# NOAA-GFDL/pace

Hardware: AMD Instinct MI355X
Metric: simulated-days/day + acoustic-step ms, C768 L79 fp64, 1/2/4/8 MI355X (higher is better)
Workload: dtype f64

## Files before the change

### pace_amd/csrc/fv3_common.h

```cpp
#pragma once
#include <type_traits>
#include <algorithm>

#include <cmath>
#include <cstdint>
#include <cstdio>
#include <cstdlib>
#include <cstring>
#include <string>
#include <vector>

#include "../../include/fv3_mi355x.h"
#include "fv3_switch.h"

#ifdef FV3_HOST_EMU
#define FV3_HD
#define FV3_DEV
typedef void *fv3_stream_t;
#else
#include <hip/hip_runtime.h>
#define FV3_HD __host__ __device__
#define FV3_DEV __device__
typedef hipStream_t fv3_stream_t;
#endif

#ifndef FV3_REAL
#define FV3_REAL double
#endif
typedef FV3_REAL Real;

#if defined(FV3_STAMPS) && !defined(FV3_HOST_EMU)
#define FV3_STAMP_RECS 16384
unsigned long long *fv3_stamp_buf();
#if defined(__HIP_DEVICE_COMPILE__)
#define FV3_STAMP_STATE unsigned st_t = (unsigned)__builtin_amdgcn_s_memtime(), st_a[6] = {0u, 0u, 0u, 0u, 0u, 0u}, st_n = 0u
#define FV3_STAMP(i)                                            \
  do {                                                          \
    __builtin_amdgcn_sched_barrier(0);                          \
    const unsigned t_ = (unsigned)__builtin_amdgcn_s_memtime(); \
    st_a[i] += t_ - st_t;                                       \
    st_t = t_;                                                  \
    if ((i) == 0) ++st_n;                                       \
    __builtin_amdgcn_sched_barrier(0);                          \
  } while (0)
#define FV3_STAMP_USE(x) asm volatile("" ::"v"(x))
#define FV3_STAMP_FLUSH(buf, kid, tid)                                          \
  do {                                                                          \
    if ((tid) == 0 && ((buf)[1] == 0ull || (buf)[1] == (kid))) {                \
      const unsigned long long slot_ = atomicAdd((buf), 1ull);                  \
      if (slot_ < FV3_STAMP_RECS) {                                             \
        unsigned long long *r_ = (buf) + 8 + slot_ * 8;                         \
        r_[0] = (kid);                                                          \
        r_[1] = st_n;                                                           \
        for (int q_ = 0; q_ < 6; ++q_) r_[2 + q_] = st_a[q_];                   \
      }                                                                         \
    }                                                                           \
  } while (0)
#else
inline void fv3_stamp_touch(unsigned long long *, unsigned long long, int) {}
#define FV3_STAMP_STATE unsigned st_n = 0u
#define FV3_STAMP(i) ((void)0)
#define FV3_STAMP_USE(x) ((void)0)
// ... 660 lines not shown
#endif
  }
  FV3_HD inline void group_sync() const {
#if !defined(FV3_HOST_EMU) && defined(__HIP_DEVICE_COMPILE__)
    asm volatile("s_waitcnt lgkmcnt(0)\n\ts_barrier" ::: "memory");
#endif
  }
  FV3_HD inline void wave_sync() const {
#if !defined(FV3_HOST_EMU) && defined(__HIP_DEVICE_COMPILE__)
    __builtin_amdgcn_fence(__ATOMIC_RELEASE, "wavefront");
    __builtin_amdgcn_wave_barrier();
    __builtin_amdgcn_fence(__ATOMIC_ACQUIRE, "wavefront");
#endif
  }
};

#ifndef FV3_HOST_EMU
template <class F>
__global__ void __launch_bounds__(256, 2) fv3_kb(GridMap m, F f) {
  extern __shared__ __attribute__((aligned(16))) char fv3_smem[];
  int bx, by, bz;
  if (!fv3_tile(m, bx, by, bz)) return;
  Blk b{(int)threadIdx.x, (int)blockDim.x, bx, by, bz};
  f(b, fv3_smem);
}
#endif

template <class F>
inline void launch_blocks(const fv3_ctx *c, fv3_stream_t s, int gx, int gy, int gz, int nthr, size_t smem_bytes, F f) {
  if (gx <= 0 || gy <= 0 || gz <= 0) return;
#ifdef FV3_HOST_EMU
  (void)c;
  (void)s;
  (void)nthr;
#pragma omp parallel
  {
    std::vector<char> smem(smem_bytes + 16);
#pragma omp for collapse(2) schedule(static)
    for (int z = 0; z < gz; ++z)
      for (int y = 0; y < gy; ++y)
        for (int x = 0; x < gx; ++x) {
          Blk b{0, 1, x, y, z};
          f(b, smem.data());
        }
  }
#else
  (void)c;
  dim3 grid;
  const GridMap m = fv3_grid(gx, gy, gz, &grid);
  hipLaunchKernelGGL(HIP_KERNEL_NAME(fv3_kb<F>), grid, dim3(nthr, 1, 1), smem_bytes, s, m, f);
#endif
}

#define FV3_WAVE 64
#ifdef FV3_HOST_EMU
#define FV3_LPT 64
#define FV3_LANES(blk, lane, l) for (int lane = 0, l = 0; lane < FV3_WAVE; ++lane, ++l)
#else
#define FV3_LPT 1
#define FV3_LANES(blk, lane, l) for (int lane = (blk).tid, l = 0; l < 1; ++l)
template <int WPE, class F>
__global__ void __launch_bounds__(FV3_WAVE) __attribute__((amdgpu_waves_per_eu(WPE, WPE))) fv3_kw(GridMap m, F f) {
  extern __shared__ __attribute__((aligned(16))) char fv3_smem[];
  int bx, by, bz;
  if (!fv3_tile(m, bx, by, bz)) return;
  Blk b{(int)threadIdx.x, FV3_WAVE, bx, by, bz};
  f(b, fv3_smem);
}
#endif

#if !defined(FV3_HOST_EMU) && defined(__HIP_DEVICE_COMPILE__)
FV3_DEV inline int fv3_dpp_shr1_i(int v) { return __builtin_amdgcn_update_dpp(0, v, 0x138, 0xf, 0xf, true); }
FV3_DEV inline int fv3_dpp_shl1_i(int v) { return __builtin_amdgcn_update_dpp(0, v, 0x130, 0xf, 0xf, true); }
FV3_DEV inline double fv3_dpp_shr1(double v) {
  return __hiloint2double(fv3_dpp_shr1_i(__double2hiint(v)), fv3_dpp_shr1_i(__double2loint(v)));
}
FV3_DEV inline double fv3_dpp_shl1(double v) {
  return __hiloint2double(fv3_dpp_shl1_i(__double2hiint(v)), fv3_dpp_shl1_i(__double2loint(v)));
}
FV3_DEV inline float fv3_dpp_shr1(float v) { return __int_as_float(fv3_dpp_shr1_i(__float_as_int(v))); }
FV3_DEV inline float fv3_dpp_shl1(float v) { return __int_as_float(fv3_dpp_shl1_i(__float_as_int(v))); }
template <int K>
FV3_DEV inline Real lane_shr_dev(Real v) {
#pragma unroll
  for (int n = 0; n < K; ++n) v = fv3_dpp_shr1(v);
  return v;
}
template <int K>
FV3_DEV inline Real lane_shl_dev(Real v) {
#pragma unroll
  for (int n = 0; n < K; ++n) v = fv3_dpp_shl1(v);
  return v;
}
#define FV3_LANE_SHR(K, arr, l, lane) lane_shr_dev<K>((arr)[l])
#define FV3_LANE_SHL(K, arr, l, lane) lane_shl_dev<K>((arr)[l])
#else
#define FV3_LANE_SHR(K, arr, l, lane) ((lane) >= (K) ? (arr)[(l) - (K)] : (Real)0)
#define FV3_LANE_SHL(K, arr, l, lane) ((lane) + (K) < FV3_WAVE ? (arr)[(l) + (K)] : (Real)0)
#endif

#ifdef FV3_HOST_EMU
#define FV3_VLPT(CPL) (FV3_WAVE * (CPL))
#define FV3_VLANES(CPL, blk, vl, l) for (int vl = 0; vl < FV3_WAVE * (CPL); ++vl) { const int l = vl; (void)l;
#define FV3_VLANES_END }
#define FV3_VSHR(CPL, K, arr, l, vl) ((vl) >= (K) ? (arr)[(l) - (K)] : (Real)0)
#define FV3_VSHL(CPL, K, arr, l, vl) ((vl) + (K) < FV3_WAVE * (CPL) ? (arr)[(l) + (K)] : (Real)0)
// ... 228 lines not shown
```

### pace_amd/csrc/fv3_dsw.hip

```cpp
#include "fv3_a2b.h"
#include "fv3_ops.h"
#include "fv3_ppm.h"

namespace {

struct FxAdv {
  Geo g;
  const Real *uc, *vc;
  long m2;
  Real dt;
  bool W, E, S, N;

  FV3_HD Real UC(int i, int j) const { return uc[IX(i, j)]; }
  FV3_HD Real VC(int i, int j) const { return vc[IX(i, j)]; }
  FV3_HD Real ut_gen(int i, int j) const {
    return (UC(i, j) - (Real)0.25 * (g.cosa_u + m2)[IX(i, j)] * (VC(i - 1, j) + VC(i, j) + VC(i - 1, j + 1) + VC(i, j + 1))) * (g.rsin_u + m2)[IX(i, j)];
  }
  FV3_HD Real vt_gen(int i, int j) const {
    return (VC(i, j) - (Real)0.25 * (g.cosa_v + m2)[IX(i, j)] * (UC(i, j - 1) + UC(i + 1, j - 1) + UC(i, j) + UC(i + 1, j))) * (g.rsin_v + m2)[IX(i, j)];
  }
  FV3_HD bool edge_col(int i) const { return (W && i == 1) || (E && i == g.npx); }
  FV3_HD bool edge_row(int j) const { return (S && j == 1) || (N && j == g.npy); }
  FV3_HD bool ut_special_row(int j) const { return (S && (j == 0 || j == 1)) || (N && (j == g.npy - 1 || j == g.npy)); }
  FV3_HD Real ut_edge(int i, int j) const {
    const Real u_ = UC(i, j);
    return u_ * dt > (Real)0 ? u_ / (g.sin_sg3 + m2)[IX(i - 1, j)] : u_ / (g.sin_sg1 + m2)[IX(i, j)];
  }
  FV3_HD Real vt_edge(int i, int j) const {
    const Real v_ = VC(i, j);
    return v_ * dt > (Real)0 ? v_ / (g.sin_sg4 + m2)[IX(i, j - 1)] : v_ / (g.sin_sg2 + m2)[IX(i, j)];
  }
  FV3_HD Real ut1(int i, int j) const {
    if (edge_col(i)) return ut_edge(i, j);
    if (ut_special_row(j)) return (Real)0;
    return ut_gen(i, j);
  }
  FV3_HD Real vt1(int i, int j) const {
    if (edge_row(j)) return vt_edge(i, j);
    return vt_gen(i, j);
  }
  FV3_HD bool in_i_rng(int i) const { return i >= (W ? 3 : 1) && i <= (E ? g.npx - 2 : g.nx + 1); }
  FV3_HD bool in_j_rng(int j) const { return j >= (S ? 3 : 1) && j <= (N ? g.npy - 2 : g.ny + 1); }
  FV3_HD bool vt_edge_col(int i) const { return (W && (i == 0 || i == 1)) || (E && (i == g.npx - 1 || i == g.npx)); }
  FV3_HD Real ut2(int i, int j) const {
    if (edge_col(i)) return ut_edge(i, j);
    if (ut_special_row(j)) {
      if (in_i_rng(i))
        return UC(i, j) - (Real)0.25 * (g.cosa_u + m2)[IX(i, j)] * (vt1(i - 1, j) + vt1(i, j) + vt1(i - 1, j + 1) + vt1(i, j + 1));
      return (Real)0;
    }
    return ut_gen(i, j);
  }
  FV3_HD Real vt2(int i, int j) const {
    if (edge_row(j)) return vt_edge(i, j);
    if (vt_edge_col(i) && in_j_rng(j))
// ... 37 lines not shown
    Real s_u = (Real)0;
    for (int n = 0; n < 4; ++n)
      if (!(pbi[n] == it && pbj[n] == j)) s_u = s_u + ut2(pbi[n], pbj[n]);
    const Real cu = (g.cosa_u + m2)[IX(it, j)], cv = (g.cosa_v + m2)[IX(pi, pj)];
    const Real damp = (Real)1 / ((Real)1 - (Real)0.0625 * cu * cv);
    return (UC(it, j) - (Real)0.25 * cu * (s_v + VC(pi, pj) - (Real)0.25 * cv * s_u)) * damp;
  }
  FV3_HD Real vt_corner(int i, int jt, bool west, bool south) const {
    const int npx = g.npx, npy = g.npy;
    const int pj = south ? 1 : npy - 1;
    const int iedge = west ? 1 : npx;
    const int nbi[4] = {i, i + 1, i, i + 1}, nbj[4] = {jt - 1, jt - 1, jt, jt};
    const int pi = (i != iedge) ? i : i + 1;
    Real s_u = (Real)0;
    for (int n = 0; n < 4; ++n)
      if (!(nbi[n] == pi && nbj[n] == pj)) s_u = s_u + ut2(nbi[n], nbj[n]);
    const int pbi[4] = {pi - 1, pi, pi - 1, pi}, pbj[4] = {pj, pj, pj + 1, pj + 1};
    Real s_v = (Real)0;
    for (int n = 0; n < 4; ++n)
      if (!(pbi[n] == i && pbj[n] == jt)) s_v = s_v + vt2(pbi[n], pbj[n]);
    const Real cv = (g.cosa_v + m2)[IX(i, jt)], cu = (g.cosa_u + m2)[IX(pi, pj)];
    const Real damp = (Real)1 / ((Real)1 - (Real)0.0625 * cu * cv);
    return (VC(i, jt) - (Real)0.25 * cv * (s_u + UC(pi, pj) - (Real)0.25 * cu * s_v)) * damp;
  }
  FV3_HD Real ut_final(int i, int j) const {
    bool w_, s_;
    if (ut_corner_target(i, j, w_, s_)) return ut_corner(i, j, w_, s_);
    return ut2(i, j);
  }
  FV3_HD Real vt_final(int i, int j) const {
    bool w_, s_;
    if (vt_corner_target(i, j, w_, s_)) return vt_corner(i, j, w_, s_);
    return vt2(i, j);
  }
};

FV3_HD inline bool fxadv_int_u(const Geo &g, int fl, int i, int j) {
  const bool W = fl & FV3_W, E = fl & FV3_E, S = fl & FV3_S, N = fl & FV3_N;
  return i >= 0 && !((W && i == 1) || (E && i == g.npx)) && !((S && (j == 0 || j == 1)) || (N && (j == g.npy - 1 || j == g.npy)));
}
FV3_HD inline bool fxadv_int_v(const Geo &g, int fl, int i, int j) {
  const bool W = fl & FV3_W, E = fl & FV3_E, S = fl & FV3_S, N = fl & FV3_N;
  return j >= 0 && !((S && j == 1) || (N && j == g.npy)) && !((W && (i == 0 || i == 1)) || (E && (i == g.npx - 1 || i == g.npx)));
}

void fxadv(fv3_ctx *c, fv3_stream_t s, const Real *uc, const Real *vc, Real *crx, Real *cry, Real *xfx, Real *yfx, Real *ut, Real *vt, Real dt, Real *cx,
           Real *cy, bool thin_ut) {
  const Geo g = c->g;
  const bool first = c->seq.acc_first;
  static const bool full_ut = fv3_sw(FV3SW_FXADV_FULL_UT);
  if (full_ut) thin_ut = false;
  const int isd = 1 - g.nh, ied = g.nx + g.nh, jsd = 1 - g.nh, jed = g.ny + g.nh;
  const int npair = (g.nz + FV3_KC - 1) / FV3_KC;
  launch3(c, s, Box{isd, ied, jsd, jed, 0, npair - 1}, [=] FV3_HD(int t, int kp, int i, int j) {
    const int fl = g.flags[t];
    const long m2 = t * g.st2;
    bool int_u = fxadv_int_u(g, fl, i, j), int_v = fxadv_int_v(g, fl, i, j);
    const unsigned p = IX(i, j);
    const bool out_x = int_u && i >= 1 && i <= g.nx + 1, out_y = int_v && j >= 1 && j <= g.ny + 1;
    const bool st_ut = !thin_ut || ((fl & FV3_W) && i <= 4) || ((fl & FV3_E) && i >= g.npx - 3) || ((fl & FV3_S) && j <= 4) || ((fl & FV3_N) && j >= g.npy - 3);
    int_u = int_u && (out_x || st_ut);
    int_v = int_v && (out_y || st_ut);
    if (!int_u && !int_v) return;
    Real cu = 0, ru = 0, rdxa_m = 0, rdxa_0 = 0, dy_ = 0, s3 = 0, s1 = 0;
    Real cv = 0, rv = 0, rdya_m = 0, rdya_0 = 0, dx_ = 0, s4 = 0, s2 = 0;
    if (int_u) {
      cu = (g.cosa_u + m2)[p];
      ru = (g.rsin_u + m2)[p];
    }
    if (out_x) {
      rdxa_m = (g.rdxa + m2)[IX(i - 1, j)];
      rdxa_0 = (g.rdxa + m2)[p];
      dy_ = (g.dy + m2)[p];
      s3 = (g.sin_sg3 + m2)[IX(i - 1, j)];
      s1 = (g.sin_sg1 + m2)[p];
    }
    if (int_v) {
      cv = (g.cosa_v + m2)[p];
      rv = (g.rsin_v + m2)[p];
    }
    if (out_y) {
      rdya_m = (g.rdya + m2)[IX(i, j - 1)];
      rdya_0 = (g.rdya + m2)[p];
      dx_ = (g.dx + m2)[p];
      s4 = (g.sin_sg4 + m2)[IX(i, j - 1)];
      s2 = (g.sin_sg2 + m2)[p];
    }
#ifndef FV3_FXADV_UNROLL
#define FV3_FXADV_UNROLL 1
#endif
#pragma unroll FV3_FXADV_UNROLL
    for (int kk = 0; kk < FV3_KC; ++kk) {
      const int k = FV3_KC * kp + kk;
      if (k > g.nz - 1) break;
      const long b = t * g.st + k * g.sk;
      const Real *ucl = uc + b, *vcl = vc + b;
      if (int_u) {
        const Real utv = (ucl[p] - (Real)0.25 * cu * (vcl[IX(i - 1, j)] + vcl[p] + vcl[IX(i - 1, j + 1)] + vcl[IX(i, j + 1)])) * ru;
        if (st_ut) (ut + b)[p] = utv;
        if (out_x) {
          const Real x = dt * utv;
          Real cr;
          if (x > (Real)0) {
            cr = x * rdxa_m;
            FV3_ST_NT((xfx + b)[p], dy_ * x * s3);
          } else {
            cr = x * rdxa_0;
            FV3_ST_NT((xfx + b)[p], dy_ * x * s1);
          }
          FV3_ST_NT((crx + b)[p], cr);
          if (cx) FV3_ST_NT((cx + b)[p], (first ? (Real)0 : (cx + b)[p]) + cr);
        }
      }
      if (int_v) {
        const Real vtv = (vcl[p] - (Real)0.25 * cv * (ucl[IX(i, j - 1)] + ucl[IX(i + 1, j - 1)] + ucl[p] + ucl[IX(i + 1, j)])) * rv;
        if (st_ut) (vt + b)[p] = vtv;
        if (out_y) {
          const Real y = dt * vtv;
          Real cr;
          if (y > (Real)0) {
            cr = y * rdya_m;
            FV3_ST_NT((yfx + b)[p], dx_ * y * s4);
          } else {
            cr = y * rdya_0;
            FV3_ST_NT((yfx + b)[p], dx_ * y * s2);
          }
          FV3_ST_NT((cry + b)[p], cr);
          if (cy) FV3_ST_NT((cy + b)[p], (first ? (Real)0 : (cy + b)[p]) + cr);
        }
      }
    }
  });
  const int nfr = std::max(ied - isd + 1, jed - jsd + 1);
  launch3(c, s, Box{0, nfr - 1, 1, 8, 0, g.nz - 1}, [=] FV3_HD(int t, int k, int a, int side) {
    const int fl = g.flags[t];
    int i, j;
    if (side <= 4) {
      i = isd + a;
      if (i > ied) return;
      j = side <= 2 ? side - 1 : g.npy - 4 + side;
      if (!(fl & (side <= 2 ? FV3_S : FV3_N))) return;
    } else {
      j = jsd + a;
      if (j > jed) return;
      i = side <= 6 ? side - 5 : g.npx - 8 + side;
      if (!(fl & (side <= 6 ? FV3_W : FV3_E))) return;
      if (((fl & FV3_S) && (j == 0 || j == 1)) || ((fl & FV3_N) && (j == g.npy - 1 || j == g.npy))) return;
    }
    const bool int_u = fxadv_int_u(g, fl, i, j), int_v = fxadv_int_v(g, fl, i, j);
    const long b = t * g.st + k * g.sk, m2 = t * g.st2;
    FxAdv f{g, uc + b, vc + b, m2, dt, (fl & FV3_W) != 0, (fl & FV3_E) != 0, (fl & FV3_S) != 0, (fl & FV3_N) != 0};
    const unsigned p = IX(i, j);
    if (i >= 0 && !int_u) {
      const Real utv = f.ut_final(i, j);
      (ut + b)[p] = utv;
      if (i >= 1 && i <= g.nx + 1) {
        const Real x = dt * utv;
        Real cr;
        if (x > (Real)0) {
          cr = x * (g.rdxa + m2)[IX(i - 1, j)];
          (xfx + b)[p] = (g.dy + m2)[p] * x * (g.sin_sg3 + m2)[IX(i - 1, j)];
        } else {
          cr = x * (g.rdxa + m2)[p];
          (xfx + b)[p] = (g.dy + m2)[p] * x * (g.sin_sg1 + m2)[p];
        }
        (crx + b)[p] = cr;
        if (cx) (cx + b)[p] = (first ? (Real)0 : (cx + b)[p]) + cr;
      }
    }
    if (j >= 0 && !int_v) {
      const Real vtv = f.vt_final(i, j);
      (vt + b)[p] = vtv;
      if (j >= 1 && j <= g.ny + 1) {
        const Real y = dt * vtv;
        Real cr;
        if (y > (Real)0) {
          cr = y * (g.rdya + m2)[IX(i, j - 1)];
          (yfx + b)[p] = (g.dx + m2)[p] * y * (g.sin_sg4 + m2)[IX(i, j - 1)];
        } else {
          cr = y * (g.rdya + m2)[p];
          (yfx + b)[p] = (g.dx + m2)[p] * y * (g.sin_sg2 + m2)[p];
        }
        (cry + b)[p] = cr;
        if (cy) (cy + b)[p] = (first ? (Real)0 : (cy + b)[p]) + cr;
      }
// ... 1097 lines not shown
```

### pace_amd/csrc/fv3_nh.hip

```cpp
#include "fv3_ops.h"
#include "fv3_math.h"
#include "fv3_agpr.h"

#define K_(arr, k) ((arr) + tb + (long)(k)*g.sk)[pix]

namespace {

struct Sim1 {
  Geo g;
  Real rgas, rgrav, p_fac, ptop;
  template <class Setup, class Finish>
  FV3_HD void run(long tb, unsigned pix, Real dt, const Real *delp, const Real *cappa, const Real *pt, const Real *w1, Real ws, Real *PM, Real *DZ, Real *W2, Real *PP,
                  Real *GAM, Real *PE, Real *wout, Setup setup, Finish finish) const {
    const int nz = g.nz;
    const Real t1g = (Real)2.0 * dt * dt, rdt = (Real)1.0 / dt, r3 = (Real)(1.0 / 3.0);
    auto DM = [&](int k) { return K_(delp, k) * rgrav; };
    auto GM = [&](int k) { return (Real)1.0 / ((Real)1.0 - K_(cappa, k)); };
    {
      Real pm_k, dz_k;
      setup(0, pm_k, dz_k);
      Real dm_m = (Real)0, dm_k = DM(0);
      Real pe_k = fv3_exp(GM(0) * fv3_log(-dm_k / dz_k * rgas * K_(pt, 0))) - pm_k;
      Real bet = (Real)0;
      K_(PP, 0) = (Real)0;
// ... 352 lines not shown
        q.v[2] = KW_(cappa, k);
        q.v[3] = KW_(PM, k);
        return q;
      };
      KWALK(4, U, false, ld, {
        const Real dm = r.v[0] * rgrav;
        const Real pe_k = K >= 1 ? A[(K - 1) * FV3_WAVE] : (Real)0;
        if (K == nz - 1) {
          p1 = (pe_k + (Real)2.0 * pe1) * r3;
        } else {
          const Real g_rat = fv3_div(dm, dm_below);
          const Real bb = (Real)2.0 * ((Real)1.0 + g_rat);
          p1 = (pe_k + bb * pe1 + g_rat * pe2) * r3 - g_rat * p1;
        }
        const Real pmk = r.v[3];
        const Real dzn = -dm * rgas * r.v[1] * fv3_exp((r.v[2] - (Real)1.0) * fv3_log(fv3_max(p_fac * pmk, p1 + pmk)));
        cl.finish(K, dzn);
        pe2 = pe1;
        pe1 = pe_k;
        dm_below = dm;
      })
    }
#undef GAM_PUT
#undef GAM_PUT_U
#undef GAM_FLUSH4
  }
};

#ifndef FV3_RIEM_GL
#define FV3_RIEM_GL 0
#endif
inline bool riem_wave_ok(const Geo &g, bool heavy = false) {
  static const int e = fv3_sw(FV3SW_RIEM_MODE);
  if (e == 1) return false;
  const size_t line = (size_t)g.nz * FV3_WAVE * sizeof(Real) * (FV3_RIEM_GL ? 2 : 1);
  if (heavy && e != 2 && line > 40 * 1024) return false;
  if ((g.nz + 2) * g.sk * (long)sizeof(Real) >= (1L << 32)) return false;
  return line <= (FV3_RIEM_GL ? 160 : 64) * 1024 && g.nz >= 3;
}
inline bool riem_gam_lds(const Geo &) { return FV3_RIEM_GL != 0; }
inline bool riem_reg_arrays(const Geo &g) {
  static const bool off = !fv3_sw(FV3SW_RIEM_REGS);
  return !off && !FV3_RIEM_GL && g.nz < (int)FV3_KREG_LEVELS;
}

#ifndef PG_KC
#define PG_KC 16
#endif

struct DzcW {
  Real top_ratio, bot_ratio;
};

}

extern "C" int fv3_update_dz_c(fv3_ctx *c, const fv3_field *zs_, const fv3_field *ut_, const fv3_field *vt_, const fv3_field *gz_, const fv3_field *ws_,
                               double dtd, void *stream) {
  return fv3_update_dz_c_from(c, zs_, ut_, vt_, gz_, gz_, ws_, dtd, stream);
}

int fv3_update_dz_c_from(fv3_ctx *c, const fv3_field *zs_, const fv3_field *ut_, const fv3_field *vt_, const fv3_field *gzin_, const fv3_field *gz_,
                         const fv3_field *ws_, double dtd, void *stream) {
  if (!c) return FV3_ERR_ARG;
  FV3_FIELD2D(zs, zs_) FV3_FIELD(ut, ut_) FV3_FIELD(vt, vt_) FV3_FIELD(gz, gz_) FV3_FIELD(gzin, gzin_) FV3_FIELD2D(ws, ws_)
  const Geo g = c->g;
  fv3_stream_t s = (fv3_stream_t)stream;
  const Real dt = (Real)dtd;
  const int nz = g.nz;
  const Real dz_min = (Real)c->cst.dz_min;
  const std::vector<double> &dp = c->dp_ref_h;
  const Real top_ratio = (Real)(dp[0] / (dp[0] + dp[1]));
  const Real bot_ratio = (Real)(dp[nz - 1] / (dp[nz - 2] + dp[nz - 1]));
  Real *gzn = c->scratch[SC_A];
  if (gzin != gz && nz >= 3) {
    launch2(c, s, Box{0, g.nx + 1, 0, g.ny + 1, 0, 0}, [=] FV3_HD(int t, int i, int j) {
      const int fl = g.flags[t];
      const long tb = t * g.st, m2 = t * g.st2;
      const unsigned pix = IX(i, j), qx1 = IX(i + 1, j), qy1 = IX(i, j + 1);
      const unsigned gw = f4_index<1>(g, fl, i - 1, j), gc1 = f4_index<1>(g, fl, i, j), ge = f4_index<1>(g, fl, i + 1, j);
      const unsigned gs = f4_index<2>(g, fl, i, j - 1), gc2 = f4_index<2>(g, fl, i, j), gn = f4_index<2>(g, fl, i, j + 1);
      const Real ar = (g.area + m2)[pix];
      Real ax0, ax1, ay0, ay1, cx0 = (Real)0, cx1 = (Real)0, cy0 = (Real)0, cy1 = (Real)0, px0 = (Real)0, px1 = (Real)0, py0 = (Real)0, py1 = (Real)0;
      {
        const Real *u1 = ut + tb + (long)(nz - 1) * g.sk, *v1 = vt + tb + (long)(nz - 1) * g.sk;
        ax0 = u1[pix];
        ax1 = u1[qx1];
        ay0 = v1[pix];
        ay1 = v1[qy1];
      }
      Real below = (Real)0;
#pragma unroll 1
      for (int k = nz; k >= 0; --k) {
        Real nx0 = (Real)0, nx1 = (Real)0, ny0 = (Real)0, ny1 = (Real)0;
        if (k >= 2) {
          const Real *u2 = ut + tb + (long)(k - 2) * g.sk, *v2 = vt + tb + (long)(k - 2) * g.sk;
          nx0 = u2[pix];
          nx1 = u2[qx1];
          ny0 = v2[pix];
          ny1 = v2[qy1];
        }
        Real x0, x1, y0, y1;
        if (k == nz) {
          x0 = ax0 + (ax0 - nx0) * bot_ratio;
          x1 = ax1 + (ax1 - nx1) * bot_ratio;
          y0 = ay0 + (ay0 - ny0) * bot_ratio;
          y1 = ay1 + (ay1 - ny1) * bot_ratio;
        } else if (k == 0) {
          x0 = cx0 + (cx0 - px0) * top_ratio;
          x1 = cx1 + (cx1 - px1) * top_ratio;
          y0 = cy0 + (cy0 - py0) * top_ratio;
          y1 = cy1 + (cy1 - py1) * top_ratio;
        } else {
          const Real d1 = g.dp_ref[k], d0 = g.dp_ref[k - 1];
          const Real int_ratio = (Real)1.0 / (d0 + d1);
          x0 = (d1 * ax0 + d0 * cx0) * int_ratio;
          x1 = (d1 * ax1 + d0 * cx1) * int_ratio;
          y0 = (d1 * ay0 + d0 * cy0) * int_ratio;
          y1 = (d1 * ay1 + d0 * cy1) * int_ratio;
        }
        const Real *gg = gzin + tb + (long)k * g.sk;
        const Real fx0 = x0 * (x0 > (Real)0 ? gg[gw] : gg[gc1]);
        const Real fx1 = x1 * (x1 > (Real)0 ? gg[gc1] : gg[ge]);
        const Real fy0 = y0 * (y0 > (Real)0 ? gg[gs] : gg[gc2]);
        const Real fy1 = y1 * (y1 > (Real)0 ? gg[gc2] : gg[gn]);
        const Real zn = (gg[pix] * ar + fx0 - fx1 + fy0 - fy1) / (ar + x0 - x1 + y0 - y1);
        Real v = zn;
        if (k == nz) {
          ws[t * g.st2 + pix] = (zs[t * g.st2 + pix] - zn) / dt;
// ... 1047 lines not shown
```

### pace_amd/csrc/fv3_switch.h

```cpp
#pragma once
#include <atomic>
#include <cstdlib>
#include <cstring>

#define FV3_SW_ONCE true
#define FV3_SW_LIVE false

enum fv3_sw_kind { FV3_SW_present, FV3_SW_off_if_0, FV3_SW_on_if_1, FV3_SW_tri, FV3_SW_word, FV3_SW_integer, FV3_SW_names };

#define FV3_SWITCH_TABLE(X) \
  X(SEG, "FV3_SEG", LIVE, integer, "", 0, "rows a marching wave owns; unset or <= 0 (default): automatic, 96 where that still fills the chip eight times over, else 64") \
  X(GRID_SPLIT, "FV3_GRID_SPLIT", ONCE, off_if_0, "", 0, "0: whole planes per XCD also for launches of few planes; default: such launches map sub-planes to the XCDs") \
  X(FRAME_LAUNCH, "FV3_FRAME_LAUNCH", ONCE, word, "split", 0, "split: one launch per boundary window; default: the four windows of a frame in one launch") \
  X(Q4_KB, "FV3_Q4_KB", ONCE, integer, "", 16, "levels of one tile an XCD walks back to back in the transport marches (level-major launches; default 16); 0: plane-major launches") \
  X(KE_KB, "FV3_KE_KB", ONCE, integer, "", 16, "the same for the corner-KE, divergence-damping and fused wind-stage marches (default 16); 0: plane-major launches") \
  X(GATHER_BATCH, "FV3_GATHER_BATCH", ONCE, off_if_0, "", 0, "0: one launch per halo gather; default: up to twelve gathers per launch") \
  X(AUX_STREAM, "FV3_AUX_STREAM", LIVE, off_if_0, "", 0, "0: everything in program order on the caller's stream; default: small launches on an auxiliary stream beside the marches (read when a context is created)") \
  X(ALT, "FV3_ALT", LIVE, names, "", 0, "named alternatives of the uncertain restatements (DESIGN section 2; the oracle reads the same variable), e.g. dz_damp_scaled,heat_dt_full; default: none") \
  X(DEBUG_FD, "FV3_DEBUG_FD", LIVE, present, "", 0, "set: the operators report on stderr which forms and level ranges they chose; default: silent") \
  X(DEBUG_DEL2, "FV3_DEBUG_DEL2", LIVE, present, "", 0, "set: the fused del2_cubed + heating reports its calls on stderr; default: silent") \
  X(TP2D_MODE, "FV3_TP2D_MODE", ONCE, word, "staged", 0, "staged: fv_tp_2d as one launch per stage (reference path, no auxiliary stream); default: the marching kernels") \
  X(DEL6_MODE, "FV3_DEL6_MODE", ONCE, word, "staged", 0, "staged: the del-n damping fluxes as one launch per stage (reference path); default: the streaming kernel") \
  X(TP2D_MARCH, "FV3_TP2D_MARCH", LIVE, word, "old", 0, "old: the round-4 single-tracer march with the del-n chain inside; default: the round-5 march that serves every tile") \
  X(TP2D_FA, "FV3_TP2D_FA", ONCE, off_if_0, "", 0, "0: the general form of the single-tracer marches with the chain inside; default: the form that takes 'order 2, on at every level' as a constant") \
  X(HORD_CONST, "FV3_HORD_CONST", ONCE, tri, "", 0, "0: PPM order at run time in every march; 1: as a constant (6) also in the two-tracer marches; default: constant in the single-tracer and wind-stage marches only") \
  X(CSW_B_GENERIC, "FV3_CSW_B_GENERIC", LIVE, present, "", 0, "set: c_sw computes every point with the generic per-point stage kernels; default: interior kernels + boundary windows") \
  X(CSW_MARCH, "FV3_CSW_MARCH", LIVE, word, "0|abc", 0, "0: c_sw's round-1 stage kernels; abc: stages A - C as a march, D and E as stage kernels; default: the whole interior as one march") \
  X(CSW_WIN_KC, "FV3_CSW_WIN_KC", ONCE, integer, "", 2, "levels one thread of c_sw's boundary-window kernels walks beside the interior march (default 2)") \
  X(CSW_WIN_OVERLAP, "FV3_CSW_WIN_OVERLAP", ONCE, off_if_0, "", 0, "0: c_sw's stage A / B windows in program order; default: on the auxiliary stream beside the march") \
  X(CSW_DEFER, "FV3_CSW_DEFER", ONCE, on_if_1, "", 0, "1: the sequencer joins c_sw's stage D / E windows only before riem_solver_c; default: c_sw waits for them") \
  X(SEQ_UAVA, "FV3_SEQ_UAVA", LIVE, word, "every", 0, "every: c_sw stores ua / va in full in every sub-step of the sequencer; default: only where a later operator reads them") \
  X(FXADV_FULL_UT, "FV3_FXADV_FULL_UT", ONCE, present, "", 0, "set: fxadv stores ut / vt everywhere inside d_sw too; default: only within 4 cells of a cube-tile edge") \
  X(DSW_SCALARS, "FV3_DSW_SCALARS", LIVE, word, "separate|quad", 0, "separate: d_sw's four scalar transports as four launches + the division kernel; quad: one four-tracer wave; default: two two-tracer marches") \
  X(DSW_DELN, "FV3_DSW_DELN", LIVE, word, "arrays", 0, "arrays: the scalars' del-n fluxes of every level from staged launches; default: the chains inside the marches above the sponge layers") \
  X(DSW_MARCH, "FV3_DSW_MARCH", LIVE, word, "old|coupled", 0, "old: the round-4 two-tracer marches; coupled: the two roles as coupled wave pairs; default: the round-5 march, one launch per role") \
  X(DSW_SPONGE_SERIAL, "FV3_DSW_SPONGE_SERIAL", ONCE, on_if_1, "", 0, "1: the sponge levels' scalar marches in program order; default: on the auxiliary stream beside the other levels") \
  X(DSW_HEAT, "FV3_DSW_HEAT", LIVE, word, "separate", 0, "separate: the damping heat in its own kernel; default: as the epilogue of the vorticity march") \
  X(DSW_VORT_DELN, "FV3_DSW_VORT_DELN", LIVE, word, "arrays", 0, "arrays: the vorticity's del-n fluxes of every level from staged launches; default: the chain inside the vorticity march") \
  X(DSW_VORT_IN_KE, "FV3_DSW_VORT_IN_KE", LIVE, on_if_1, "", 0, "1: the corner-KE march also forms the cell vorticity under its corners; default: the vorticity kernel forms all of it") \
  X(DSW_WINDSTAGE, "FV3_DSW_WINDSTAGE", LIVE, word, "staged", 0, "staged: every level of d_sw's wind stage through the staged kernels; default: the fused wind-stage march above the sponge layers") \
  X(KE_STAGED, "FV3_KE_STAGED", ONCE, present, "", 0, "set: the corner kinetic energy as stage kernels (profiling; switches the fused wind stage off); default: the marching kernel") \
  X(DIVDAMP_STAGED, "FV3_DIVDAMP_STAGED", ONCE, present, "", 0, "set: the divergence damping as one launch per iteration (profiling; switches the fused wind stage off); default: the marching iteration") \
  X(DSW_SPONGE_WIND, "FV3_DSW_SPONGE_WIND", LIVE, word, "serial", 0, "serial: the sponge levels' wind chain in program order; default: on the auxiliary stream beside the fused wind stage") \
  X(DSW_SIDE, "FV3_DSW_SIDE", LIVE, word, "copy", 0, "copy: separate copies of the winds on the segment / strip boundaries for the damping heat; default: the wind stage stores them") \
  X(DSW_WIND_OVERLAP, "FV3_DSW_WIND_OVERLAP", ONCE, on_if_1, "", 0, "1: d_sw's wind branch on the auxiliary stream beside the scalar marches; default: in program order behind them") \
  X(RIEM_MODE, "FV3_RIEM_MODE", ONCE, word, "columns|wave", 0, "columns: thread-per-column Riemann solvers; wave: the LDS-line wave form also for deep columns; default: wave form unless riem_solver3's line exceeds 40 KB") \
  X(RIEM_REGS, "FV3_RIEM_REGS", ONCE, off_if_0, "", 0, "0: the wave solvers' gam through the scratch field; default: in the accumulation registers") \
  X(SEQ_DELZ, "FV3_SEQ_DELZ", LIVE, word, "every", 0, "every: riem_solver3 stores delz in every sub-step of the sequencer; default: only in the last one of a call") \
  X(NH_PGF, "FV3_NH_PGF", LIVE, word, "staged", 0, "staged: nh_p_grad as four a2b_ord4 launches + the level-walking update; default: one marching kernel") \
  X(EP_ONE_LAUNCH, "FV3_EP_ONE_LAUNCH", ONCE, off_if_0, "", 0, "0: edge_profile's four solves as four launches; default: one launch") \
  X(EDGE_PROFILE_GENERIC, "FV3_EDGE_PROFILE_GENERIC", ONCE, present, "", 0, "set: edge_profile's generic thread-per-column form; default: the wave forms") \
  X(EDGE_PROFILE_REG, "FV3_EDGE_PROFILE_REG", ONCE, present, "", 0, "set: edge_profile's register-resident column form; default: the wave forms") \
  X(EDGE_PROFILE_LDS, "FV3_EDGE_PROFILE_LDS", ONCE, present, "", 0, "set: edge_profile's wave form with the level count at run time also for 79 / 127 levels; default: their own instantiations") \
  X(DZ_DELN, "FV3_DZ_DELN", LIVE, word, "arrays", 0, "arrays: update_dz_d's del-n fluxes of every interface from one staged launch; default: the chain inside the transport march") \
  X(DZ_SCAN, "FV3_DZ_SCAN", LIVE, word, "separate", 0, "separate: update_dz_d's closing scan as its own kernel also inside the sequencer; default: left to riem_solver3's pre-sweep there") \
  X(DEL2_FUSED, "FV3_DEL2_FUSED", LIVE, off_if_0, "", 0, "0: del2_cubed and the diffusive heating as the two staged operators; default: one fused pass") \
  X(DEL2_HEAT, "FV3_DEL2_HEAT", LIVE, word, "fused", 0, "fused: the heating as the epilogue of the third del2 iteration; default: its own launch on the smoothed field") \
  X(FRAME_FIRST, "FV3_FRAME_FIRST", LIVE, tri, "", 0, "1: operators that feed a halo update compute the frame first; set to anything else: never; default: only with a message transport") \
  X(ACC_STORE, "FV3_ACC_STORE", LIVE, off_if_0, "", 0, "0: flux accumulators zeroed, then read-modify-write in every sub-step; default: the first sub-step of a call stores") \
  X(ACC_DEFER, "FV3_ACC_DEFER", LIVE, off_if_0, "", 0, "0: cx / cy read-modify-write in every sub-step; default: summed once per call (read when a context first allocates the slots)") \
  X(PINGPONG, "FV3_PINGPONG", LIVE, off_if_0, "", 0, "0: d_sw copies its new scalars back in place; default: the sequencer alternates two buffer sets (read when a context first allocates them)") \
  X(GZ_FIRST, "FV3_GZ_FIRST", LIVE, word, "copy", 0, "copy: the reference's order at the start of a call (gz filled, copied to zh, updated in place); default: heights straight into zh") \
  X(SEQ_KEEP_DIVGD, "FV3_SEQ_KEEP_DIVGD", LIVE, present, "", 0, "set: d_sw leaves the iterated divergence in divgd inside the sequencer; default: not stored there (nothing reads it)")

#define FV3_SW_ENUM_(id, env, policy, kind, words, dflt, what) FV3SW_##id,
enum fv3_sw_id { FV3_SWITCH_TABLE(FV3_SW_ENUM_) FV3SW_COUNT };
#undef FV3_SW_ENUM_

struct fv3_sw_row {
  const char *env;
  bool once;
  fv3_sw_kind kind;
  const char *words;
  int dflt;
  const char *what;
};
#define FV3_SW_ROW_(id, env, policy, kind, words, dflt, what) {env, FV3_SW_##policy, FV3_SW_##kind, words, dflt, what},
inline constexpr fv3_sw_row fv3_sw_rows[FV3SW_COUNT] = {FV3_SWITCH_TABLE(FV3_SW_ROW_)};
#undef FV3_SW_ROW_

inline int fv3_sw_word(const char *words, const char *w) {
  const size_t n = strlen(w);
  int i = 1;
  for (const char *p = words; *p; ++i) {
    const char *q = strchr(p, '|');
    const size_t len = q ? (size_t)(q - p) : strlen(p);
    if (len == n && !strncmp(p, w, n)) return i;
    p += len + (q ? 1 : 0);
  }
  return 0;
}

inline int fv3_sw_parse(const fv3_sw_row &r, const char *v) {
  switch (r.kind) {
    case FV3_SW_present:
    case FV3_SW_names: return v != nullptr;
    case FV3_SW_off_if_0: return !(v && v[0] == '0');
    case FV3_SW_on_if_1: return v && v[0] == '1';
    case FV3_SW_tri: return !v ? -1 : v[0] == '0' ? 0 : v[0] == '1' ? 1 : 2;
    case FV3_SW_word: return v ? fv3_sw_word(r.words, v) : 0;
    case FV3_SW_integer: return v ? atoi(v) : r.dflt;
  }
  return 0;
}

inline std::atomic<long long> fv3_sw_cache[FV3SW_COUNT];

inline int fv3_sw(fv3_sw_id id) {
  const fv3_sw_row &r = fv3_sw_rows[id];
  if (!r.once) return fv3_sw_parse(r, getenv(r.env));
  long long seen = fv3_sw_cache[id].load(std::memory_order_acquire);
  if (!seen) {
    const long long mine = (1LL << 32) | (long long)(unsigned)fv3_sw_parse(r, getenv(r.env));
    if (fv3_sw_cache[id].compare_exchange_strong(seen, mine)) seen = mine;
  }
// ... 17 lines not shown
```

Baseline: 211.7.

## Stage fxadv and update_dz_c stencil inputs through double-buffered LDS tiles

Adds a generic tile-kernel launcher that stages halo'd input planes into double-buffered LDS per level, prefetching the next level into registers while the current one is computed. fxadv's interior kernel now uses it by default, reading uc/vc from LDS instead of issuing repeated global neighbour loads. update_dz_c gets an optional tile form behind a switch that is off by default. The change cuts redundant global traffic, at the cost of barriers per level, more LDS use and lower occupancy, plus extra register state for per-point constants.

```diff
diff --git a/pace_amd/csrc/fv3_common.h b/pace_amd/csrc/fv3_common.h
--- a/pace_amd/csrc/fv3_common.h
+++ b/pace_amd/csrc/fv3_common.h
@@ -8,6 +8,8 @@
 #include <cstdlib>
 #include <cstring>
 #include <string>
+#include <tuple>
+#include <utility>
 #include <vector>
 
 #include "../../include/fv3_mi355x.h"
@@ -774,6 +776,227 @@
 #endif
 }
 
+#ifndef FV3_HOST_EMU
+template <int R, class F>
+__global__ void __launch_bounds__(64 * R) fv3_k3r(Box b, int nkc, GridMap m, F f) {
+  int bx, by, kz;
+  if (!fv3_tile(m, bx, by, kz)) return;
+  const int i = b.i0 + (int)(bx * 64 + threadIdx.x);
+  const int j = b.j0 + (int)(by * R + threadIdx.y);
+  const int t = kz / nkc;
+  const int k = b.k0 + (kz - t * nkc);
+  if (i <= b.i1 && j <= b.j1) f(t, k, i, j);
+}
+#endif
+template <int R, class F>
+inline void launch3_rows(const fv3_ctx *c, fv3_stream_t s, Box b, F f) {
+#ifdef FV3_HOST_EMU
+  launch3(c, s, b, f);
+#else
+  const int ni = b.i1 - b.i0 + 1, nj = b.j1 - b.j0 + 1, nk = b.k1 - b.k0 + 1;
+  if (ni <= 0 || nj <= 0 || nk <= 0) return;
+  dim3 block(64, R, 1), grid;
+  const GridMap m = fv3_grid((ni + 63) / 64, (nj + R - 1) / R, c->g.nsub * nk, &grid);
+  hipLaunchKernelGGL(HIP_KERNEL_NAME(fv3_k3r<R, F>), grid, block, 0, s, b, nk, m, f);
+#endif
+}
+#ifndef FV3_HOST_EMU
+template <int R, class F>
+__global__ void __launch_bounds__(64 * R) fv3_k2r(Box b, GridMap m, F f) {
+  int bx, by, t;
+  if (!fv3_tile(m, bx, by, t)) return;
+  const int i = b.i0 + (int)(bx * 64 + threadIdx.x);
+  const int j = b.j0 + (int)(by * R + threadIdx.y);
+  if (i <= b.i1 && j <= b.j1) f(t, i, j);
+}
+#endif
+template <int R, class F>
+inline void launch2_rows(const fv3_ctx *c, fv3_stream_t s, Box b, F f) {
+#ifdef FV3_HOST_EMU
+  launch2(c, s, b, f);
+#else
+  const int ni = b.i1 - b.i0 + 1, nj = b.j1 - b.j0 + 1;
+  if (ni <= 0 || nj <= 0) return;
+  dim3 block(64, R, 1), grid;
+  const GridMap m = fv3_grid((ni + 63) / 64, (nj + R - 1) / R, c->g.nsub, &grid);
+  hipLaunchKernelGGL(HIP_KERNEL_NAME(fv3_k2r<R, F>), grid, block, 0, s, b, m, f);
+#endif
+}
+
+template <int W_, int E_, int S_, int N_>
+struct TileHalo {
+  static constexpr int W = W_, E = E_, S = S_, N = N_;
+};
+template <class... H>
+struct TileHalos {
+  typedef std::tuple<H...> tuple;
+  static constexpr int NIN = (int)sizeof...(H);
+};
+struct TileLevels {
+  int kc, nlev, kfirst, kdir;
+};
+template <int R, class HL>
+struct TileLay {
+  static constexpr int NIN = HL::NIN, NTHR = 64 * R;
+  template <int n>
+  using H = std::tuple_element_t<n, typename HL::tuple>;
+  template <int n>
+  static constexpr int pitch() { return 64 + H<n>::W + H<n>::E; }
+  template <int n>
+  static constexpr int size() { return pitch<n>() * (R + H<n>::S + H<n>::N); }
+  template <int n>
+  static constexpr int off() {
+    if constexpr (n == 0)
+      return 0;
+    else
+      return off<n - 1>() + size<n - 1>();
+  }
+  template <int n>
+  static constexpr int nq() { return (size<n>() + NTHR - 1) / NTHR; }
+  template <int n>
+  static constexpr int qbase() {
+    if constexpr (n == 0)
+      return 0;
+    else
+      return qbase<n - 1>() + nq<n - 1>();
+  }
+  static constexpr int total() { return off<NIN>(); }
+  static constexpr size_t lds_bytes() { return 2 * (size_t)total() * sizeof(Real); }
+};
+template <int N0, int N1, class F>
+FV3_HD inline void fv3_static_for(F &&f) {
+  if constexpr (N0 < N1) {
+    f(std::integral_constant<int, N0>{});
+    fv3_static_for<N0 + 1, N1>(f);
+  }
+}
+template <int R, class HL>
+struct TileView {
+  typedef TileLay<R, HL> L;
+  const Real *buf;
+  int tx, ty;
+  template <int n>
+  FV3_HD Real at(int di, int dj) const {
+    return buf[L::template off<n>() + (ty + L::template H<n>::S + dj) * L::template pitch<n>() + (tx + L::template H<n>::W + di)];
+  }
+};
+template <int R, class HL, int n, class G>
+FV3_HD inline bool fv3_tile_src(const G &g, int i0, int j0, int e, unsigned &goff) {
+  typedef TileLay<R, HL> L;
+  typedef typename L::template H<n> H;
+  const int r = e / L::template pitch<n>(), cc = e - r * L::template pitch<n>();
+  const int si = i0 - H::W + cc + g.o, sj = j0 - H::S + r + g.o;
+  goff = (unsigned)(sj * g.sj32 + si);
+  return e < L::template size<n>() && si >= 0 && si < g.ni && sj >= 0 && sj < g.nj;
+}
+#ifndef FV3_HOST_EMU
+struct TileGeo {
+  int o, sj32, ni, nj;
+};
+#ifdef FV3_TILE_WPE
+#define FV3_TILE_OCC __attribute__((amdgpu_waves_per_eu(FV3_TILE_WPE, FV3_TILE_WPE)))
+#else
+#define FV3_TILE_OCC
+#endif
+template <int R, class HL, class Pre, class Plane, class Step>
+__global__ void __launch_bounds__(64 * R) FV3_TILE_OCC fv3_k3t(Box b, int nchunk, TileLevels lv, TileGeo g, GridMap m, Pre pre, Plane plane, Step step) {
+  typedef TileLay<R, HL> L;
+  __shared__ __attribute__((aligned(16))) Real lds[2 * L::total()];
+  int bx, by, kz;
+  if (!fv3_tile(m, bx, by, kz)) return;
+  const int t = kz / nchunk, q = b.k0 + (kz - t * nchunk);
+  const int tx = (int)threadIdx.x, ty = (int)threadIdx.y, tid = ty * 64 + tx;
+  const int i0 = b.i0 + bx * 64, j0 = b.j0 + by * R, i = i0 + tx, j = j0 + ty;
+  const bool act = i <= b.i1 && j <= b.j1;
+  constexpr int NQ = L::template qbase<L::NIN>();
+  unsigned goff[NQ];
+  bool gok[NQ];
+  Real val[NQ];
+  fv3_static_for<0, L::NIN>([&](auto nc) {
+    constexpr int n = decltype(nc)::value, base = L::template qbase<n>();
+#pragma unroll
+    for (int qq = 0; qq < L::template nq<n>(); ++qq) gok[base + qq] = fv3_tile_src<R, HL, n>(g, i0, j0, tid + qq * L::NTHR, goff[base + qq]);
+  });
+  auto fetch = [&](int k) {
+    fv3_static_for<0, L::NIN>([&](auto nc) {
+      constexpr int n = decltype(nc)::value, base = L::template qbase<n>();
+      const Real *p = plane(n, t, k);
+#pragma unroll
+      for (int qq = 0; qq < L::template nq<n>(); ++qq) val[base + qq] = p && gok[base + qq] ? FV3_EL(p, goff[base + qq]) : (Real)0;
+    });
+  };
+  decltype(pre(0, 0, 0)) st{};
+  if (act) st = pre(t, i, j);
+  const int kb = q * lv.kc, nl = lv.nlev - kb < lv.kc ? lv.nlev - kb : lv.kc;
+  if (nl > 0) fetch(lv.kfirst + lv.kdir * kb);
+#pragma unroll 1
+  for (int kk = 0; kk < nl; ++kk) {
+    const int k = lv.kfirst + lv.kdir * (kb + kk);
+    Real *buf = lds + (kk & 1) * L::total();
+    fv3_static_for<0, L::NIN>([&](auto nc) {
+      constexpr int n = decltype(nc)::value, base = L::template qbase<n>();
+#pragma unroll
+      for (int qq = 0; qq < L::template nq<n>(); ++qq) {
+        const int e = tid + qq * L::NTHR;
+        if (e < L::template size<n>()) buf[L::template off<n>() + e] = val[base + qq];
+      }
+    });
+    if (kk + 1 < nl) fetch(k + lv.kdir);
+    asm volatile("s_waitcnt lgkmcnt(0)\n\ts_barrier" ::: "memory");
+    if (act) step(st, t, k, i, j, TileView<R, HL>{buf, tx, ty});
+  }
+}
+#endif
+template <int R, class HL, class Pre, class Plane, class Step>
+inline void launch3_tile(const fv3_ctx *c, fv3_stream_t s, Box b, TileLevels lv, Pre pre, Plane plane, Step step) {
+  typedef TileLay<R, HL> L;
+  static_assert(L::lds_bytes() <= 64 * 1024, "a tile kernel's two buffers are static LDS (64 KB at most; two workgroups per CU fit below 80 KB)");
+  const int ni = b.i1 - b.i0 + 1, nj = b.j1 - b.j0 + 1, nchunk = b.k1 - b.k0 + 1;
+  if (ni <= 0 || nj <= 0 || nchunk <= 0 || lv.nlev <= 0) return;
+  const int gx = (ni + 63) / 64, gy = (nj + R - 1) / R;
+#ifdef FV3_HOST_EMU
+  (void)s;
+  const Geo &g = c->g;
+  const int nsub = g.nsub;
+#pragma omp parallel
+  {
+    std::vector<Real> tile(L::total());
+    std::vector<decltype(pre(0, 0, 0))> st(L::NTHR);
+#pragma omp for collapse(2) schedule(static)
+    for (int t = 0; t < nsub; ++t)
+      for (int q = b.k0; q <= b.k1; ++q)
+        for (int by = 0; by < gy; ++by)
+          for (int bx = 0; bx < gx; ++bx) {
+            const int i0 = b.i0 + bx * 64, j0 = b.j0 + by * R;
+            for (int tid = 0; tid < L::NTHR; ++tid) {
+              const int i = i0 + (tid & 63), j = j0 + (tid >> 6);
+              if (i <= b.i1 && j <= b.j1) st[tid] = pre(t, i, j);
+            }
+            for (int kk = 0; kk < lv.kc && q * lv.kc + kk < lv.nlev; ++kk) {
+              const int k = lv.kfirst + lv.kdir * (q * lv.kc + kk);
+              fv3_static_for<0, L::NIN>([&](auto nc) {
+                constexpr int n = decltype(nc)::value;
+                const Real *p = plane(n, t, k);
+                for (int e = 0; e < L::template size<n>(); ++e) {
+                  unsigned goff;
+                  tile[L::template off<n>() + e] = fv3_tile_src<R, HL, n>(g, i0, j0, e, goff) && p ? p[goff] : (Real)0;
+                }
+              });
+              for (int tid = 0; tid < L::NTHR; ++tid) {
+                const int i = i0 + (tid & 63), j = j0 + (tid >> 6);
+                if (i <= b.i1 && j <= b.j1) step(st[tid], t, k, i, j, TileView<R, HL>{tile.data(), tid & 63, tid >> 6});
+              }
+            }
+          }
+  }
+#else
+  dim3 block(64, R, 1), grid;
+  const GridMap m = fv3_grid(gx, gy, c->g.nsub * nchunk, &grid);
+  const TileGeo tg{c->g.o, c->g.sj32, c->g.ni, c->g.nj};
+  hipLaunchKernelGGL(HIP_KERNEL_NAME(fv3_k3t<R, HL, Pre, Plane, Step>), grid, block, 0, s, b, nchunk, lv, tg, m, pre, plane, step);
+#endif
+}
+
 #define FV3_WAVE 64
 #ifdef FV3_HOST_EMU
 #define FV3_LPT 64
diff --git a/pace_amd/csrc/fv3_dsw.hip b/pace_amd/csrc/fv3_dsw.hip
--- a/pace_amd/csrc/fv3_dsw.hip
+++ b/pace_amd/csrc/fv3_dsw.hip
@@ -1,6 +1,10 @@
 #include "fv3_a2b.h"
 #include "fv3_ops.h"
 #include "fv3_ppm.h"
+
+#ifndef FV3_FXADV_TILE_R
+#define FV3_FXADV_TILE_R 8
+#endif
 
 namespace {
 
@@ -144,7 +148,12 @@
   if (full_ut) thin_ut = false;
   const int isd = 1 - g.nh, ied = g.nx + g.nh, jsd = 1 - g.nh, jed = g.ny + g.nh;
   const int npair = (g.nz + FV3_KC - 1) / FV3_KC;
+  if (fv3_sw_is(FV3SW_FXADV_FORM, "point"))
+#ifdef FV3_FXADV_ROWS
+  launch3_rows<FV3_FXADV_ROWS>(c, s, Box{isd, ied, jsd, jed, 0, npair - 1}, [=] FV3_HD(int t, int kp, int i, int j) {
+#else
   launch3(c, s, Box{isd, ied, jsd, jed, 0, npair - 1}, [=] FV3_HD(int t, int kp, int i, int j) {
+#endif
     const int fl = g.flags[t];
     const long m2 = t * g.st2;
     bool int_u = fxadv_int_u(g, fl, i, j), int_v = fxadv_int_v(g, fl, i, j);
@@ -223,6 +232,92 @@
       }
     }
   });
+  else {
+    struct St {
+      bool int_u, int_v, out_x, out_y, st_ut;
+      unsigned p;
+      Real cu, ru, rdxa_m, rdxa_0, dy_, s3, s1, cv, rv, rdya_m, rdya_0, dx_, s4, s2;
+    };
+    typedef TileHalos<TileHalo<0, 1, 1, 0>, TileHalo<1, 0, 0, 1>> HL;
+    launch3_tile<FV3_FXADV_TILE_R, HL>(
+        c, s, Box{isd, ied, jsd, jed, 0, npair - 1}, TileLevels{FV3_KC, g.nz, 0, 1},
+        [=] FV3_HD(int t, int i, int j) {
+          St q{};
+          const int fl = g.flags[t];
+          const long m2 = t * g.st2;
+          q.int_u = fxadv_int_u(g, fl, i, j);
+          q.int_v = fxadv_int_v(g, fl, i, j);
+          const unsigned p = IX(i, j);
+          q.p = p;
+          q.out_x = q.int_u && i >= 1 && i <= g.nx + 1;
+          q.out_y = q.int_v && j >= 1 && j <= g.ny + 1;
+          q.st_ut = !thin_ut || ((fl & FV3_W) && i <= 4) || ((fl & FV3_E) && i >= g.npx - 3) || ((fl & FV3_S) && j <= 4) || ((fl & FV3_N) && j >= g.npy - 3);
+          q.int_u = q.int_u && (q.out_x || q.st_ut);
+          q.int_v = q.int_v && (q.out_y || q.st_ut);
+          if (q.int_u) {
+            q.cu = (g.cosa_u + m2)[p];
+            q.ru = (g.rsin_u + m2)[p];
+          }
+          if (q.out_x) {
+            q.rdxa_m = (g.rdxa + m2)[IX(i - 1, j)];
+            q.rdxa_0 = (g.rdxa + m2)[p];
+            q.dy_ = (g.dy + m2)[p];
+            q.s3 = (g.sin_sg3 + m2)[IX(i - 1, j)];
+            q.s1 = (g.sin_sg1 + m2)[p];
+          }
+          if (q.int_v) {
+            q.cv = (g.cosa_v + m2)[p];
+            q.rv = (g.rsin_v + m2)[p];
+          }
+          if (q.out_y) {
+            q.rdya_m = (g.rdya + m2)[IX(i, j - 1)];
+            q.rdya_0 = (g.rdya + m2)[p];
+            q.dx_ = (g.dx + m2)[p];
+            q.s4 = (g.sin_sg4 + m2)[IX(i, j - 1)];
+            q.s2 = (g.sin_sg2 + m2)[p];
+          }
+          return q;
+        },
+        [=] FV3_HD(int n, int t, int k) -> const Real * { return (n == 0 ? uc : vc) + (t * g.st + k * g.sk); },
+        [=] FV3_HD(St & q, int t, int k, int, int, const TileView<FV3_FXADV_TILE_R, HL> &v) {
+          const long b = t * g.st + k * g.sk;
+          const unsigned p = q.p;
+          if (q.int_u) {
+            const Real utv = (v.at<0>(0, 0) - (Real)0.25 * q.cu * (v.at<1>(-1, 0) + v.at<1>(0, 0) + v.at<1>(-1, 1) + v.at<1>(0, 1))) * q.ru;
+            if (q.st_ut) (ut + b)[p] = utv;
+            if (q.out_x) {
+              const Real x = dt * utv;
+              Real cr;
+              if (x > (Real)0) {
+                cr = x * q.rdxa_m;
+                FV3_ST_NT((xfx + b)[p], q.dy_ * x * q.s3);
+              } else {
+                cr = x * q.rdxa_0;
+                FV3_ST_NT((xfx + b)[p], q.dy_ * x * q.s1);
+              }
+              FV3_ST_NT((crx + b)[p], cr);
+              if (cx) FV3_ST_NT((cx + b)[p], (first ? (Real)0 : (cx + b)[p]) + cr);
+            }
+          }
+          if (q.int_v) {
+            const Real vtv = (v.at<1>(0, 0) - (Real)0.25 * q.cv * (v.at<0>(0, -1) + v.at<0>(1, -1) + v.at<0>(0, 0) + v.at<0>(1, 0))) * q.rv;
+            if (q.st_ut) (vt + b)[p] = vtv;
+            if (q.out_y) {
+              const Real y = dt * vtv;
+              Real cr;
+              if (y > (Real)0) {
+                cr = y * q.rdya_m;
+                FV3_ST_NT((yfx + b)[p], q.dx_ * y * q.s4);
+              } else {
+                cr = y * q.rdya_0;
+                FV3_ST_NT((yfx + b)[p], q.dx_ * y * q.s2);
+              }
+              FV3_ST_NT((cry + b)[p], cr);
+              if (cy) FV3_ST_NT((cy + b)[p], (first ? (Real)0 : (cy + b)[p]) + cr);
+            }
+          }
+        });
+  }
   const int nfr = std::max(ied - isd + 1, jed - jsd + 1);
   launch3(c, s, Box{0, nfr - 1, 1, 8, 0, g.nz - 1}, [=] FV3_HD(int t, int k, int a, int side) {
     const int fl = g.flags[t];
diff --git a/pace_amd/csrc/fv3_nh.hip b/pace_amd/csrc/fv3_nh.hip
--- a/pace_amd/csrc/fv3_nh.hip
+++ b/pace_amd/csrc/fv3_nh.hip
@@ -428,6 +428,112 @@
   Real top_ratio, bot_ratio;
 };
 
+#ifndef FV3_DZC_TILE_R
+#define FV3_DZC_TILE_R 8
+#endif
+
+void fv3_update_dz_c_tile(fv3_ctx *c, fv3_stream_t s, const Real *zs, const Real *ut, const Real *vt, const Real *gzin, Real *gz, Real *ws, Real dt, Real dz_min,
+                          Real top_ratio, Real bot_ratio) {
+  const Geo g = c->g;
+  const int nz = g.nz;
+  struct St {
+    unsigned pix;
+    bool rem;
+    Real ar, below, ax0, ax1, ay0, ay1, cx0, cx1, cy0, cy1, px0, px1, py0, py1;
+  };
+  typedef TileHalos<TileHalo<1, 1, 1, 1>, TileHalo<0, 1, 0, 0>, TileHalo<0, 0, 0, 1>> HL;
+  launch3_tile<FV3_DZC_TILE_R, HL>(
+      c, s, Box{0, g.nx + 1, 0, g.ny + 1, 0, 0}, TileLevels{nz + 1, nz + 1, nz, -1},
+      [=] FV3_HD(int t, int i, int j) {
+        St q{};
+        const int fl = g.flags[t];
+        const long tb = t * g.st, m2 = t * g.st2;
+        const unsigned pix = IX(i, j), qx1 = IX(i + 1, j), qy1 = IX(i, j + 1);
+        q.pix = pix;
+        q.rem = f4_index<1>(g, fl, i - 1, j) != IX(i - 1, j) || f4_index<1>(g, fl, i, j) != pix || f4_index<1>(g, fl, i + 1, j) != qx1 ||
+                f4_index<2>(g, fl, i, j - 1) != IX(i, j - 1) || f4_index<2>(g, fl, i, j) != pix || f4_index<2>(g, fl, i, j + 1) != qy1;
+        q.ar = (g.area + m2)[pix];
+        const Real *u1 = ut + tb + (long)(nz - 1) * g.sk, *v1 = vt + tb + (long)(nz - 1) * g.sk;
+        q.ax0 = u1[pix];
+        q.ax1 = u1[qx1];
+        q.ay0 = v1[pix];
+        q.ay1 = v1[qy1];
+        return q;
+      },
+      [=] FV3_HD(int n, int t, int k) -> const Real * {
+        if (n == 0) return gzin + (t * g.st + (long)k * g.sk);
+        if (k < 2) return nullptr;
+        return (n == 1 ? ut : vt) + (t * g.st + (long)(k - 2) * g.sk);
+      },
+      [=] FV3_HD(St & q, int t, int k, int i, int j, const TileView<FV3_DZC_TILE_R, HL> &v) {
+        const long tb = t * g.st;
+        const unsigned pix = q.pix;
+        Real nx0 = (Real)0, nx1 = (Real)0, ny0 = (Real)0, ny1 = (Real)0;
+        if (k >= 2) {
+          nx0 = v.at<1>(0, 0);
+          nx1 = v.at<1>(1, 0);
+          ny0 = v.at<2>(0, 0);
+          ny1 = v.at<2>(0, 1);
+        }
+        Real x0, x1, y0, y1;
+        if (k == nz) {
+          x0 = q.ax0 + (q.ax0 - nx0) * bot_ratio;
+          x1 = q.ax1 + (q.ax1 - nx1) * bot_ratio;
+          y0 = q.ay0 + (q.ay0 - ny0) * bot_ratio;
+          y1 = q.ay1 + (q.ay1 - ny1) * bot_ratio;
+        } else if (k == 0) {
+          x0 = q.cx0 + (q.cx0 - q.px0) * top_ratio;
+          x1 = q.cx1 + (q.cx1 - q.px1) * top_ratio;
+          y0 = q.cy0 + (q.cy0 - q.py0) * top_ratio;
+          y1 = q.cy1 + (q.cy1 - q.py1) * top_ratio;
+        } else {
+          const Real d1 = g.dp_ref[k], d0 = g.dp_ref[k - 1];
+          const Real int_ratio = (Real)1.0 / (d0 + d1);
+          x0 = (d1 * q.ax0 + d0 * q.cx0) * int_ratio;
+          x1 = (d1 * q.ax1 + d0 * q.cx1) * int_ratio;
+          y0 = (d1 * q.ay0 + d0 * q.cy0) * int_ratio;
+          y1 = (d1 * q.ay1 + d0 * q.cy1) * int_ratio;
+        }
+        const Real zc = v.at<0>(0, 0);
+        Real zw = v.at<0>(-1, 0), zc1 = zc, ze = v.at<0>(1, 0), zs_ = v.at<0>(0, -1), zc2 = zc, zn_ = v.at<0>(0, 1);
+        if (q.rem) {
+          const int fl = g.flags[t];
+          const Real *gg = gzin + tb + (long)k * g.sk;
+          zw = gg[f4_index<1>(g, fl, i - 1, j)];
+          zc1 = gg[f4_index<1>(g, fl, i, j)];
+          ze = gg[f4_index<1>(g, fl, i + 1, j)];
+          zs_ = gg[f4_index<2>(g, fl, i, j - 1)];
+          zc2 = gg[f4_index<2>(g, fl, i, j)];
+          zn_ = gg[f4_index<2>(g, fl, i, j + 1)];
+        }
+        const Real fx0 = x0 * (x0 > (Real)0 ? zw : zc1);
+        const Real fx1 = x1 * (x1 > (Real)0 ? zc1 : ze);
+        const Real fy0 = y0 * (y0 > (Real)0 ? zs_ : zc2);
+        const Real fy1 = y1 * (y1 > (Real)0 ? zc2 : zn_);
+        const Real zn = (zc * q.ar + fx0 - fx1 + fy0 - fy1) / (q.ar + x0 - x1 + y0 - y1);
+        Real val = zn;
+        if (k == nz) {
+          ws[t * g.st2 + pix] = (zs[t * g.st2 + pix] - zn) / dt;
+        } else {
+          val = fv3_max(zn, q.below + dz_min);
+        }
+        (gz + tb + (long)k * g.sk)[pix] = val;
+        q.below = val;
+        q.px0 = q.cx0;
+        q.px1 = q.cx1;
+        q.py0 = q.cy0;
+        q.py1 = q.cy1;
+        q.cx0 = q.ax0;
+        q.cx1 = q.ax1;
+        q.cy0 = q.ay0;
+        q.cy1 = q.ay1;
+        q.ax0 = nx0;
+        q.ax1 = nx1;
+        q.ay0 = ny0;
+        q.ay1 = ny1;
+      });
+}
+
 }
 
 extern "C" int fv3_update_dz_c(fv3_ctx *c, const fv3_field *zs_, const fv3_field *ut_, const fv3_field *vt_, const fv3_field *gz_, const fv3_field *ws_,
@@ -449,7 +555,15 @@
   const Real bot_ratio = (Real)(dp[nz - 1] / (dp[nz - 2] + dp[nz - 1]));
   Real *gzn = c->scratch[SC_A];
   if (gzin != gz && nz >= 3) {
+    if (fv3_sw_is(FV3SW_DZC_FORM, "tile")) {
+      fv3_update_dz_c_tile(c, s, zs, ut, vt, gzin, gz, ws, dt, dz_min, top_ratio, bot_ratio);
+      return fv3_post(c, s, "update_dz_c");
+    }
+#ifdef FV3_DZC_ROWS
+    launch2_rows<FV3_DZC_ROWS>(c, s, Box{0, g.nx + 1, 0, g.ny + 1, 0, 0}, [=] FV3_HD(int t, int i, int j) {
+#else
     launch2(c, s, Box{0, g.nx + 1, 0, g.ny + 1, 0, 0}, [=] FV3_HD(int t, int i, int j) {
+#endif
       const int fl = g.flags[t];
       const long tb = t * g.st, m2 = t * g.st2;
       const unsigned pix = IX(i, j), qx1 = IX(i + 1, j), qy1 = IX(i, j + 1);
diff --git a/pace_amd/csrc/fv3_switch.h b/pace_amd/csrc/fv3_switch.h
--- a/pace_amd/csrc/fv3_switch.h
+++ b/pace_amd/csrc/fv3_switch.h
@@ -31,6 +31,7 @@
   X(CSW_DEFER, "FV3_CSW_DEFER", ONCE, on_if_1, "", 0, "1: the sequencer joins c_sw's stage D / E windows only before riem_solver_c; default: c_sw waits for them") \
   X(SEQ_UAVA, "FV3_SEQ_UAVA", LIVE, word, "every", 0, "every: c_sw stores ua / va in full in every sub-step of the sequencer; default: only where a later operator reads them") \
   X(FXADV_FULL_UT, "FV3_FXADV_FULL_UT", ONCE, present, "", 0, "set: fxadv stores ut / vt everywhere inside d_sw too; default: only within 4 cells of a cube-tile edge") \
+  X(FXADV_FORM, "FV3_FXADV_FORM", LIVE, word, "point|tile", 0, "point: fxadv's interior kernel reads uc / vc per point on 64 x 4 workgroups; tile or default: it stages them through one LDS tile per 64 x 8 workgroup") \
   X(DSW_SCALARS, "FV3_DSW_SCALARS", LIVE, word, "separate|quad", 0, "separate: d_sw's four scalar transports as four launches + the division kernel; quad: one four-tracer wave; default: two two-tracer marches") \
   X(DSW_DELN, "FV3_DSW_DELN", LIVE, word, "arrays", 0, "arrays: the scalars' del-n fluxes of every level from staged launches; default: the chains inside the marches above the sponge layers") \
   X(DSW_MARCH, "FV3_DSW_MARCH", LIVE, word, "old|coupled", 0, "old: the round-4 two-tracer marches; coupled: the two roles as coupled wave pairs; default: the round-5 march, one launch per role") \
@@ -61,6 +62,7 @@
   X(ACC_DEFER, "FV3_ACC_DEFER", LIVE, off_if_0, "", 0, "0: cx / cy read-modify-write in every sub-step; default: summed once per call (read when a context first allocates the slots)") \
   X(PINGPONG, "FV3_PINGPONG", LIVE, off_if_0, "", 0, "0: d_sw copies its new scalars back in place; default: the sequencer alternates two buffer sets (read when a context first allocates them)") \
   X(GZ_FIRST, "FV3_GZ_FIRST", LIVE, word, "copy", 0, "copy: the reference's order at the start of a call (gz filled, copied to zh, updated in place); default: heights straight into zh") \
+  X(DZC_FORM, "FV3_DZC_FORM", LIVE, word, "point|tile", 0, "tile: update_dz_c's one-kernel zh -> gz form stages zh / ut / vt through LDS tiles of 64 x 8 points; point or default: the column kernel on 64 x 4 workgroups") \
   X(SEQ_KEEP_DIVGD, "FV3_SEQ_KEEP_DIVGD", LIVE, present, "", 0, "set: d_sw leaves the iterated divergence in divgd inside the sequencer; default: not stored there (nothing reads it)")
 
 #define FV3_SW_ENUM_(id, env, policy, kind, words, dflt, what) FV3SW_##id,
```

After: 211.1. Within noise of the previous version (-0.3%).
